# lowc1012/tensorflow-distributed-example

Measured on AMD Instinct MI355X. Metric: images/sec (whole node) MNIST CNN at 1/2/4/8 MI355X; step time ms, higher is better.
Workload: dtype fp32; 1 GPU; model=mnist_cnn, global_batch=64, per_gpu_batch=64, parallelism=dp1, replicas=1, replicas_per_process=1, distinct_devices=1, graphs_per_execution=1, steps_per_execution=3, warmup_steps_run=6360, optimizer=SGD(lr=0.001), plan=fused_convnet, allreduce=none, hipgraph=True, grad_buckets=1, optimizer_placement=in_step_kernels

## Files before the change

### csrc/include/tde_convnet.h

```cpp
#pragma once
#include "tde_optim.h"
#include "tde_xgmi.h"

namespace tde {
namespace cnet {

constexpr int CC = 32;
constexpr int HD = 64;
constexpr int NW = 16;

struct FwdArgs {
  const float* x; const float* wc; const float* bc;
  const void* W1; int ldw1;
  float* hpre;
  void* Pt; int ldPt;
  uint64_t* amax; int lda;
  int B, H, W;
  long long* stamps;
  int w1_rows;
  const int* pend;
  const float *gwc, *gbc, *mwc, *mbc, *vwc, *vbc;
  const long long* iterations;
  OptHyper h;
  unsigned long long* inc_iter;
  int hrep; long long hrep_stride;
  int grep; long long grep_stride;
  unsigned long long* fly_count;
  const float *hsrc_w2, *hsrc_b2, *hsrc_b1;
  float* hsnap;
  int hC;
};

__device__ __forceinline__ void fwd_snap_head(const FwdArgs& a, int nthreads) {
  if (!a.hsnap || blockIdx.x != 0 || blockIdx.y != 0) return;
  const int C = a.hC, n = HD + HD * C + C;
  for (int i = threadIdx.x; i < n; i += nthreads) {
    float v;
    if (i < HD) v = a.hsrc_b1 ? a.hsrc_b1[i] : 0.f;
    else if (i < HD + HD * C) v = a.hsrc_w2[i - HD];
    else v = a.hsrc_b2[i - HD - HD * C];
    a.hsnap[i] = v;
  }
}

constexpr int XR = 6, XW = 32;
__host__ __device__ constexpr int fwd_istride(int W) { return XR * W + ((2 - (XR * W) % 64) + 64) % 64; }
constexpr int kConvW = CC * 10;
constexpr int kXrBytes = 64 * (XR * XW + 64) * 4;

__device__ __forceinline__ void fwd_stage_x(const FwdArgs& a, float* xr, int b0, int py0, int nrows, int nthreads) {
  const int W = a.W, H = a.H;
  const int istride = fwd_istride(W);
  const int n4 = nrows * W / 4;
  constexpr int kU = 8;
  for (int i0 = threadIdx.x; i0 < 64 * n4; i0 += kU * nthreads) {
    float4 v[kU];
#pragma unroll
    for (int u = 0; u < kU; ++u) {
      const int i = i0 + u * nthreads, bl = i / n4, q = i - bl * n4;
      v[u] = float4{0.f, 0.f, 0.f, 0.f};
      if (i < 64 * n4 && b0 + bl < a.B)
        v[u] = *reinterpret_cast<const float4*>(a.x + (size_t)(b0 + bl) * H * W + (size_t)(2 * py0) * W + q * 4);
    }
#pragma unroll
    for (int u = 0; u < kU; ++u) {
      const int i = i0 + u * nthreads, bl = i / n4, q = i - bl * n4;
      if (i < 64 * n4) {
        float2* d2 = reinterpret_cast<float2*>(xr + bl * istride + q * 4);
        d2[0] = float2{v[u].x, v[u].y};
        d2[1] = float2{v[u].z, v[u].w};
      }
    }
  }
}

__device__ __forceinline__ void fwd_stage_conv(const FwdArgs& a, float* wcs, int nthreads) {
  for (int i = threadIdx.x; i < kConvW; i += nthreads) {
    const bool isb = i >= 9 * CC;
    const int j = isb ? i - 9 * CC : i;
    float w = isb ? a.bc[j] : a.wc[j];
    if (a.pend) {
      const float* gp = isb ? a.gbc + j : a.gwc + j;
      float gv[kMaxGrep];
#pragma unroll
      for (int r = 0; r < kMaxGrep; ++r) gv[r] = (r == 0 || r < a.grep) ? gp[r * a.grep_stride] : 0.f;
      float g = gv[0];
#pragma unroll
      for (int r = 1; r < kMaxGrep; ++r) g += gv[r];
      float m = 0.f, v = 0.f;
      if (a.h.kind != kOptSGD) m = isb ? a.mbc[j] : a.mwc[j];
      if (a.h.kind == kOptAdam) v = isb ? a.vbc[j] : a.vwc[j];
      const long long t = a.h.kind == kOptAdam ? *a.iterations : 0;
      if (*a.pend) w = opt_step(a.h, opt_lr_t(a.h, t), w, g, m, v);
    }
    wcs[i] = w;
  }
}

struct ConvW8 {
  float4 wlo[9], whi[9], blo, bhi;
  __device__ __forceinline__ void load(const float* wcs, int c0) {
#pragma unroll
    for (int t = 0; t < 9; ++t) {
      wlo[t] = *reinterpret_cast<const float4*>(wcs + t * CC + c0);
      whi[t] = *reinterpret_cast<const float4*>(wcs + t * CC + c0 + 4);
    }
    blo = *reinterpret_cast<const float4*>(wcs + 9 * CC + c0);
    bhi = *reinterpret_cast<const float4*>(wcs + 9 * CC + c0 + 4);
  }
};

__device__ __forceinline__ float f4get(float4 q, int k) { return k == 0 ? q.x : (k == 1 ? q.y : (k == 2 ? q.z : q.w)); }

__device__ __forceinline__ void conv_pool8(const float* xb, int W, const ConvW8& cw, float out[8], uint64_t& packed) {
  float patch[16];
#pragma unroll
  for (int r = 0; r < 4; ++r) {
    const float2 u = *reinterpret_cast<const float2*>(xb + r * W);
    const float2 v = *reinterpret_cast<const float2*>(xb + r * W + 2);
    patch[r * 4 + 0] = u.x; patch[r * 4 + 1] = u.y; patch[r * 4 + 2] = v.x; patch[r * 4 + 3] = v.y;
  }
  packed = 0;
#pragma unroll
  for (int cc = 0; cc < 8; ++cc) {
    float wt[9];
#pragma unroll
    for (int t = 0; t < 9; ++t) wt[t] = f4get(cc < 4 ? cw.wlo[t] : cw.whi[t], cc & 3);
    const float bcv = f4get(cc < 4 ? cw.blo : cw.bhi, cc & 3);
    float best = -3.0e38f;
    int bi = 0;
#pragma unroll
    for (int q = 0; q < 4; ++q) {
      const int dy = q >> 1, dx = q & 1;
      float z = bcv;
#pragma unroll
      for (int ky = 0; ky < 3; ++ky)
#pragma unroll
        for (int kx = 0; kx < 3; ++kx) z = fmaf(patch[(dy + ky) * 4 + dx + kx], wt[ky * 3 + kx], z);
      if (z > best) { best = z; bi = q; }
    }
    out[cc] = fmaxf(best, 0.f);
    packed |= (uint64_t)(best > 0.f ? (unsigned)bi : 0xFFu) << (8 * cc);
  }
}

struct BwdArgs {
  const float* x; const uint64_t* amax; int lda;
  const float* hpre;
  float* hzero;
  int hrep; long long hrep_stride;
  float* cpart;
  const float* b1; const float* W2; const float* b2; int C; int pre_relu;
  const int* labels;
  float scale;
  float* metrics;
// ... 17 lines not shown
  int* pend_set;
  XgPush push;
};

template <int NPER>
struct FlatPrefetch {
  int e[NPER];
  float w[NPER], g[NPER], m[NPER], v[NPER];
  __device__ __forceinline__ void load(const FlatApply& f, int tid, int nt) {
#pragma unroll
    for (int k = 0; k < NPER; ++k) {
      int idx = tid + k * nt;
      e[k] = -1;
      for (int r = 0; r < f.nr; ++r) {
        if (idx < f.n[r]) {
          e[k] = f.lo[r] + idx;
          break;
        }
        idx -= f.n[r];
      }
      w[k] = g[k] = m[k] = v[k] = 0.f;
      if (e[k] >= 0) {
        w[k] = f.w[e[k]];
        g[k] = flat_grad(f, e[k]);
        if (f.h.kind != kOptSGD) m[k] = f.m[e[k]];
        if (f.h.kind == kOptAdam) v[k] = f.v[e[k]];
      }
    }
  }
  __device__ __forceinline__ void apply(const FlatApply& f, long long t) {
    const float lr_t = opt_lr_t(f.h, t);
#pragma unroll
    for (int k = 0; k < NPER; ++k) {
      if (e[k] < 0) continue;
      f.w[e[k]] = opt_step(f.h, lr_t, w[k], g[k], m[k], v[k]);
      flat_grad_zero(f, e[k]);
      if (f.h.kind != kOptSGD) f.m[e[k]] = m[k];
      if (f.h.kind == kOptAdam) f.v[e[k]] = v[k];
    }
  }
};

__device__ __forceinline__ f32x4 mfma_f32x4(float a, float b, f32x4 c) {
  return __builtin_amdgcn_mfma_f32_16x16x4f32(a, b, c, 0, 0, 0);
}

constexpr int HS = HD + 4;
constexpr int DLS = 17, W2S = 17;
constexpr int kHeadScratch = 64 * HS * 4 + 12 * 64 * 4 * 4 + 64 * DLS * 4;
struct HeadLds {
  float* hs;
  float* part;
  float* dls;
  float* w2s;
  float* b2s;
  int* labs;
  __device__ __forceinline__ static HeadLds carve(unsigned char* scratch, unsigned char* w2, unsigned char* b2,
                                                  unsigned char* lab) {
    HeadLds l;
    l.hs = reinterpret_cast<float*>(scratch);
    l.part = reinterpret_cast<float*>(scratch + 64 * HS * 4);
    l.dls = reinterpret_cast<float*>(scratch + 64 * HS * 4 + 12 * 64 * 4 * 4);
    l.w2s = reinterpret_cast<float*>(w2);
    l.b2s = reinterpret_cast<float*>(b2);
    l.labs = reinterpret_cast<int*>(lab);
    return l;
  }
};
constexpr int kW2Bytes = HD * W2S * 4, kB2Bytes = 16 * 4, kLabBytes = 64 * 4;

__device__ __forceinline__ void head_load_w2(const BwdArgs& a, const HeadLds& l, int tid) {
  const int u = tid >> 4, c = tid & 15;
  l.w2s[u * W2S + c] = c < a.C ? a.W2[u * a.C + c] : 0.f;
  if (tid < 16) l.b2s[tid] = tid < a.C ? a.b2[tid] : 0.f;
}

__device__ __forceinline__ void zero_other_parity(const BwdArgs& a, int tid) {
  const int n4 = (int)(((a.hrep - 1) * a.hrep_stride + (long long)a.B * HD) / 4);
  const int per = (n4 + gridDim.x - 1) / gridDim.x, beg = blockIdx.x * per;
  const int end = min(n4, beg + per);
  for (int i = beg + tid; i < end; i += 1024) reinterpret_cast<float4*>(a.hzero)[i] = float4{0.f, 0.f, 0.f, 0.f};
}

__device__ __forceinline__ float4 load_hpre(const BwdArgs& a, int row, int c4) {
  constexpr int kMaxRep = 8;
  if (a.hrep > kMaxRep) {
    float4 s = {0.f, 0.f, 0.f, 0.f};
    for (int r = 0; r < a.hrep; ++r) {
      const float4 v = *reinterpret_cast<const float4*>(a.hpre + (size_t)r * a.hrep_stride + (size_t)row * HD + c4);
      s.x += v.x; s.y += v.y; s.z += v.z; s.w += v.w;
    }
    return s;
  }
  float4 v[kMaxRep];
#pragma unroll
  for (int r = 0; r < kMaxRep; ++r)
    v[r] = r < a.hrep ? *reinterpret_cast<const float4*>(a.hpre + (size_t)r * a.hrep_stride + (size_t)row * HD + c4)
                      : float4{0.f, 0.f, 0.f, 0.f};
  float4 s = v[0];
#pragma unroll
  for (int r = 1; r < kMaxRep; ++r) {
    s.x += v[r].x; s.y += v[r].y; s.z += v[r].z; s.w += v[r].w;
  }
  return s;
}

__device__ __forceinline__ void head_stage(const BwdArgs& a, float4 hv, float4 b1v, int hr, int hc4, int nb,
                                           float* hs) {
  float4 h = float4{hv.x + b1v.x, hv.y + b1v.y, hv.z + b1v.z, hv.w + b1v.w};
  if (a.pre_relu) h = float4{fmaxf(h.x, 0.f), fmaxf(h.y, 0.f), fmaxf(h.z, 0.f), fmaxf(h.w, 0.f)};
  if (hr >= nb) h = float4{0.f, 0.f, 0.f, 0.f};
  *reinterpret_cast<float4*>(hs + hr * HS + hc4) = h;
}

__device__ __forceinline__ void head_logits_ce(const BwdArgs& a, int nb, const HeadLds& l, int lane, int wave,
                                               float& la, float& ca, float& na) {
  const int fr = lane & 15, fq = lane >> 4, C = a.C;
  f32x4 lg = {0.f, 0.f, 0.f, 0.f};
  {
    const int rt = wave & 3, kq = wave >> 2;
#pragma unroll
    for (int k = kq * 16; k < kq * 16 + 16; k += 4)
      lg = mfma_f32x4(l.hs[(rt * 16 + fr) * HS + k + fq], l.w2s[(k + fq) * W2S + fr], lg);
    if (kq > 0) *reinterpret_cast<f32x4*>(l.part + (((kq - 1) * 4 + rt) * 64 + lane) * 4) = lg;
  }
  lds_barrier();
  if (wave < 4) {
    const int rt = wave;
#pragma unroll
    for (int q = 0; q < 3; ++q) {
      const f32x4 pv = *reinterpret_cast<const f32x4*>(l.part + ((q * 4 + rt) * 64 + lane) * 4);
      lg[0] += pv[0]; lg[1] += pv[1]; lg[2] += pv[2]; lg[3] += pv[3];
    }
#pragma unroll
    for (int i = 0; i < 4; ++i) {
      const int r = rt * 16 + fq * 4 + i;
      const bool valid = r < nb;
      const bool cv = fr < C;
      const float z = cv ? lg[i] + l.b2s[fr] : -3.0e38f;
      const float m = row16_max(z);
      const float e = cv ? __expf(z - m) : 0.f;
      const float s = row16_sum(e);
      const float pr = e / s;
      const int label = l.labs[r];
      const int amx = row16_min(cv && z == m ? fr : 64);
      const float zl = __shfl(z, (lane & ~15) | (label & 15), 64);
      if (valid && fr == 0) {
        la += __logf(s) + m - zl;
        ca += (amx == label) ? 1.f : 0.f;
        na += 1.f;
      }
      l.dls[r * DLS + fr] = (valid && cv) ? (pr - (fr == label ? 1.f : 0.f)) * a.scale : 0.f;
    }
  }
  lds_barrier();
}

__device__ __forceinline__ f32x4 head_dh(const BwdArgs& a, int nb, const HeadLds& l, int lane, int wave) {
  const int fr = lane & 15, fq = lane >> 4, rt = wave >> 2, ut = wave & 3;
  f32x4 gh = {0.f, 0.f, 0.f, 0.f};
#pragma unroll
  for (int k = 0; k < 16; k += 4)
    gh = mfma_f32x4(l.dls[(rt * 16 + fr) * DLS + k + fq], l.w2s[(ut * 16 + fr) * W2S + k + fq], gh);
  const int j = ut * 16 + fr;
#pragma unroll
  for (int i = 0; i < 4; ++i) {
    const int r = rt * 16 + fq * 4 + i;
    if ((a.pre_relu && !(l.hs[r * HS + j] > 0.f)) || r >= nb) gh[i] = 0.f;
  }
  return gh;
}

template <int MODE>
__device__ __forceinline__ void head_workgroup(const BwdArgs& a, const HeadLds& l, float* db1p) {
  const int lane = threadIdx.x & 63, wave = threadIdx.x >> 6, tid = threadIdx.x;
  const int fr = lane & 15, fq = lane >> 4, C = a.C;
  const int hr = tid >> 4, hc4 = (tid & 15) * 4;
  const float4 b1v = a.b1 ? *reinterpret_cast<const float4*>(a.b1 + hc4) : float4{0.f, 0.f, 0.f, 0.f};

  long long e[4] = {-1, -1, -1, -1};
  if (wave < 4 && fr < C) {
#pragma unroll
    for (int i = 0; i < 4; ++i) e[i] = a.off_w2 + (long long)(wave * 16 + fq * 4 + i) * C + fr;
  } else if (wave == 4 && fq == 0 && fr < C) {
    e[0] = a.off_b2 + fr;
  } else if (wave == 5 && a.off_b1 >= 0) {
    e[0] = a.off_b1 + lane;
  }
  float hwv[4] = {0.f, 0.f, 0.f, 0.f}, hmv[4] = {0.f, 0.f, 0.f, 0.f}, hvv[4] = {0.f, 0.f, 0.f, 0.f};
  long long t_it = 0;
  FlatPrefetch<1> cp;
  int cpend = 0;
  if (MODE != 0) {
    t_it = *a.iterations;
#pragma unroll
    for (int i = 0; i < 4; ++i) {
      if (e[i] < 0) continue;
      hwv[i] = a.hw[e[i]];
      if (MODE == 2 && a.h.kind != kOptSGD) hmv[i] = a.hm[e[i]];
      if (MODE == 2 && a.h.kind == kOptAdam) hvv[i] = a.hv[e[i]];
    }
    if (a.commit.nr > 0) {
      cpend = *a.commit.pend;
      cp.load(a.commit, tid, 1024);
    }
  }

  f32x4 gw = {0.f, 0.f, 0.f, 0.f};
  float db1acc = 0.f, db2acc = 0.f, la = 0.f, ca = 0.f, na = 0.f;
  for (int b0 = 0; b0 < a.B; b0 += 64) {
    const int nb = min(64, a.B - b0);
    float4 hv = {0.f, 0.f, 0.f, 0.f};
    if (hr < nb) hv = load_hpre(a, b0 + hr, hc4);
    const int lab = (tid < nb) ? a.labels[b0 + tid] : 0;
    head_stage(a, hv, b1v, hr, hc4, nb, l.hs);
    if (tid < 64) l.labs[tid] = lab;
    lds_barrier();
    head_logits_ce(a, nb, l, lane, wave, la, ca, na);
    const f32x4 gh = head_dh(a, nb, l, lane, wave);
    db1acc += (gh[0] + gh[1]) + (gh[2] + gh[3]);
    if (wave < 4) {
#pragma unroll
      for (int k = 0; k < 64; k += 4) gw = mfma_f32x4(l.hs[(k + fq) * HS + wave * 16 + fr], l.dls[(k + fq) * DLS + fr], gw);
    } else if (wave == 4) {
#pragma unroll 4
      for (int r = fq * 16; r < fq * 16 + 16; ++r) db2acc += l.dls[r * DLS + fr];
    }
    lds_barrier();
  }
  db1acc += __shfl_xor(db1acc, 16, 64);
  db1acc += __shfl_xor(db1acc, 32, 64);
  if (fq == 0) db1p[(wave >> 2) * 64 + (wave & 3) * 16 + fr] = db1acc;
  db2acc += __shfl_xor(db2acc, 16, 64);
  db2acc += __shfl_xor(db2acc, 32, 64);
  if (wave < 4) {
    la = rows4_sum(la);
    ca = rows4_sum(ca);
    na = rows4_sum(na);
    if (a.metrics && lane == 0 && na > 0.f) {
      atomicAdd(a.metrics + 0, la);
      atomicAdd(a.metrics + 1, ca);
      atomicAdd(a.metrics + 2, na);
    }
  }
  lds_barrier();
  float gv[4] = {0.f, 0.f, 0.f, 0.f};
  float* gdst[4] = {nullptr, nullptr, nullptr, nullptr};
  if (wave < 4 && fr < C) {
#pragma unroll
    for (int i = 0; i < 4; ++i) {
      gv[i] = gw[i];
      gdst[i] = a.dW2 ? a.dW2 + (size_t)(wave * 16 + fq * 4 + i) * C + fr : nullptr;
    }
  } else if (wave == 4 && fq == 0 && fr < C) {
    gv[0] = db2acc;
    gdst[0] = a.db2 ? a.db2 + fr : nullptr;
  } else if (wave == 5 && a.b1) {
    gv[0] = (db1p[lane] + db1p[64 + lane]) + (db1p[128 + lane] + db1p[192 + lane]);
    gdst[0] = a.db1 ? a.db1 + lane : nullptr;
  }
  if (MODE == 0) {
#pragma unroll
    for (int i = 0; i < 4; ++i)
      if (gdst[i]) *gdst[i] += gv[i];
    stamp(a.stamps, 7);
    return;
  }
  const float lr_t = opt_lr_t(a.h, t_it);
#pragma unroll
  for (int i = 0; i < 4; ++i) {
    if (e[i] < 0) continue;
    float m = hmv[i], v = hvv[i];
    a.hw[e[i]] = opt_step(a.h, lr_t, hwv[i], gv[i], m, v);
    if (MODE == 2 && a.h.kind != kOptSGD) a.hm[e[i]] = m;
    if (MODE == 2 && a.h.kind == kOptAdam) a.hv[e[i]] = v;
  }
  if (cpend) cp.apply(a.commit, t_it - 1);
  if (tid == 0) {
    if (cpend) *a.commit.pend = 0;
    if (cpend && a.commit.count) atomicAdd(a.commit.count, 1ull);
    if (a.pend_set) *a.pend_set = 1;
    if (a.iter_prev) *a.iter_prev = t_it;
  }
  stamp(a.stamps, 7);
}

__device__ __forceinline__ void conv_grad_reduce(const BwdArgs& a, const f32x4 accr[2], float* red, int lane, int wave) {
  const int fr = lane & 15, fq = lane >> 4, tid = threadIdx.x;
#pragma unroll
  for (int ct = 0; ct < 2; ++ct)
#pragma unroll
    for (int r = 0; r < 4; ++r) red[((size_t)wave * 16 + fq * 4 + r) * CC + ct * 16 + fr] = accr[ct][r];
  lds_barrier();
  if (tid < 10 * CC) {
    const int tap = tid / CC, c = tid - tap * CC;
    float s = 0.f;
#pragma unroll
    for (int w = 0; w < NW; ++w) s += red[((size_t)w * 16 + tap) * CC + c];
    if (a.cpart) a.cpart[(size_t)blockIdx.x * 10 * CC + tid] = s;
    else {
      const long long ro = a.crep > 1 ? (long long)(blockIdx.x % a.crep) * a.crep_stride : 0;
      if (tap < 9) {
        if (a.dwc) atomicAdd(a.dwc + ro + tap * CC + c, s);
      } else if (a.dbc) {
        atomicAdd(a.dbc + ro + c, s);
      }
    }
  }
}

}
}


struct TdeStepOpt {
  int kind;
  float lr, mom, b1, b2, eps;
  float *w, *g, *m, *v;
  const long long* iterations;
  int* pend;
  int grep; long long grep_stride;
  unsigned long long* fly_count;
  const float *hsrc_w2, *hsrc_b2, *hsrc_b1;
  float* hsnap;
  int hC;
};

struct TdeBwdOpt {
  int kind;
  float lr, mom, b1, b2, eps;
  float *w, *m, *v;
  long long off_w1, off_w2, off_b2, off_b1;
  void* W1c; int ldw1c;
  const long long* iterations;
  long long* iter_prev;
  tde::FlatApply commit;
  int* pend_set;
  int crep; long long crep_stride;
};

namespace tde {
namespace cnet {

inline OptHyper hyper_of(const TdeStepOpt* o) { return OptHyper{o->kind, o->lr, o->mom, o->b1, o->b2, o->eps}; }
inline bool opt_ok(const TdeStepOpt* o) {
  return o->w && o->g && o->iterations && (o->kind == kOptSGD || o->m) && (o->kind != kOptAdam || o->v) &&
         (!o->hsnap || (o->hsrc_w2 && o->hsrc_b2 && o->hC >= 1 && o->hC <= 16 && !((uintptr_t)o->hsnap & 15)));
}

inline void fill_fwd_opt(FwdArgs& a, const TdeStepOpt* opt, long long off_wc, long long off_bc, long long* inc_iter,
                         int hrep, long long hrep_stride) {
  a.inc_iter = (unsigned long long*)inc_iter;
  a.hrep = hrep > 0 ? hrep : 1;
  a.hrep_stride = hrep_stride;
  if (opt) {
    a.pend = opt->pend;
    a.gwc = opt->g + off_wc;
    a.gbc = opt->g + off_bc;
// ... 95 lines not shown
```

### csrc/kernels/convnet_f32.hip

```cpp
#include "tde_convnet.h"

namespace tde {
using namespace cnet;

constexpr int FG = 4;
constexpr int FB = 16;
constexpr int AS32 = 168;
constexpr int GS32 = 72;
constexpr int DPS32 = 40;
static_assert(FG == 4 && FB == 16, "the forward's lane maps are written for 4 positions x 16 images");

__host__ __device__ constexpr int fwd32_istride(int W) { return XR * W + ((4 - (XR * W) % 64) + 64) % 64; }
constexpr int kXr32Bytes = FB * (XR * XW + 64) * 4;
constexpr int kFwd32Lds = FB * AS32 * 4 + kXr32Bytes + kConvW * 4;

__device__ __forceinline__ int k8_col(int fq, int i) { return fq * 8 + 4 * ((i + fq) & 1); }
__device__ __forceinline__ int k16_col(int fq, int i) { return fq * 16 + 4 * ((i + fq) & 3); }

__device__ __forceinline__ void fwd32_stage_x(const FwdArgs& a, float* xr, int b0, int py0, int nrows) {
  const int W = a.W, H = a.H;
  const int istride = fwd32_istride(W);
  const int n4 = nrows * W / 4;
  constexpr int kU = 3;
  for (int i0 = threadIdx.x; i0 < FB * n4; i0 += kU * 256) {
    float4 v[kU];
#pragma unroll
    for (int u = 0; u < kU; ++u) {
      const int i = i0 + u * 256, bl = i / n4, q = i - bl * n4;
      v[u] = float4{0.f, 0.f, 0.f, 0.f};
      if (i < FB * n4 && b0 + bl < a.B)
        v[u] = *reinterpret_cast<const float4*>(a.x + (size_t)(b0 + bl) * H * W + (size_t)(2 * py0) * W + q * 4);
    }
#pragma unroll
    for (int u = 0; u < kU; ++u) {
      const int i = i0 + u * 256, bl = i / n4, q = i - bl * n4;
      if (i < FB * n4) *reinterpret_cast<float4*>(xr + bl * istride + q * 4) = v[u];
    }
  }
}

__global__ __launch_bounds__(256) void convnet32_fwd_kernel(FwdArgs a) {
  constexpr int NT = 256;
  extern __shared__ __attribute__((aligned(16))) unsigned char fsm[];
  float* As = reinterpret_cast<float*>(fsm);
  float* xr = reinterpret_cast<float*>(fsm + FB * AS32 * 4);
  float* wcs = reinterpret_cast<float*>(fsm + FB * AS32 * 4 + kXr32Bytes);
  stamp(a.stamps, 0);
  if (a.inc_iter && blockIdx.x == 0 && blockIdx.y == 0 && threadIdx.x == 0) atomicAdd(a.inc_iter, 1ull);
  if (a.fly_count && a.pend && blockIdx.x == 0 && blockIdx.y == 0 && threadIdx.x == 0 && *a.pend)
    atomicAdd(a.fly_count, 1ull);
  fwd_snap_head(a, NT);
  const int lane = threadIdx.x & 63, wave = __builtin_amdgcn_readfirstlane(threadIdx.x >> 6);
  const int fr = lane & 15, fq = lane >> 4;
  const int W = a.W, H = a.H;
  const int Wp = (W - 2) / 2, Hp = (H - 2) / 2, P = Hp * Wp;
  const int p0 = blockIdx.x * FG;
  const int b0 = blockIdx.y * FB;
  const int py0 = p0 / Wp;
  const int nrows = min(XR, H - 2 * py0);
  const float* W1 = reinterpret_cast<const float*>(a.W1);
  float* Pt = reinterpret_cast<float*>(a.Pt);

  const int nt = wave;
  float wfr[FG][8];
#pragma unroll
  for (int ks = 0; ks < FG; ++ks) {
    const int kp = p0 + ks;
#pragma unroll
    for (int i = 0; i < 2; ++i)
#pragma unroll
      for (int j = 0; j < 4; ++j)
        wfr[ks][4 * i + j] = kp < P ? W1[(size_t)(kp * CC + k8_col(fq, i) + j) * a.ldw1 + nt * 16 + fr] : 0.f;
  }
  fwd32_stage_x(a, xr, b0, py0, nrows);
  fwd_stage_conv(a, wcs, NT);
  stamp(a.stamps, 1);
  lds_barrier();

  const int cg = wave, c0 = cg * 8;
  ConvW8 cw;
  cw.load(wcs, c0);
  const int p = p0 + fq, b = b0 + fr;
  const bool pok = p < P, bok = b < a.B;
  float out[8];
  if (bok && pok) {
    const int py = p / Wp, px = p - py * Wp;
    uint64_t packed;
    conv_pool8(xr + fr * fwd32_istride(W) + (2 * (py - py0)) * W + 2 * px, W, cw, out, packed);
    if (a.amax) a.amax[((size_t)p * (CC / 8) + cg) * a.lda + b] = packed;
  } else {
#pragma unroll
    for (int cc = 0; cc < 8; ++cc) out[cc] = 0.f;
  }
  if (pok && Pt && (bok || b < a.ldPt)) {
#pragma unroll
    for (int cc = 0; cc < 8; ++cc) Pt[(size_t)(p * CC + c0 + cc) * a.ldPt + b] = out[cc];
  }
  {
    float* dst = As + fr * AS32 + fq * CC + c0;
    *reinterpret_cast<float4*>(dst) = float4{out[0], out[1], out[2], out[3]};
    *reinterpret_cast<float4*>(dst + 4) = float4{out[4], out[5], out[6], out[7]};
  }
  stamp(a.stamps, 2);
  lds_barrier();
  stamp(a.stamps, 3);

  float* const hrow = a.hpre + (size_t)(blockIdx.x % a.hrep) * a.hrep_stride;
  f32x4 acc[FG];
#pragma unroll
  for (int ks = 0; ks < FG; ++ks) acc[ks] = f32x4{0.f, 0.f, 0.f, 0.f};
#pragma unroll
  for (int i = 0; i < 2; ++i) {
    float4 av[FG];
#pragma unroll
    for (int ks = 0; ks < FG; ++ks)
      av[ks] = *reinterpret_cast<const float4*>(As + fr * AS32 + ks * CC + k8_col(fq, i));
#pragma unroll
    for (int e = 0; e < 4; ++e)
#pragma unroll
      for (int ks = 0; ks < FG; ++ks) acc[ks] = mfma_f32x4(f4get(av[ks], e), wfr[ks][4 * i + e], acc[ks]);
  }
#pragma unroll
  for (int r = 0; r < 4; ++r) {
    const int row = b0 + fq * 4 + r;
    const float s = ((acc[0][r] + acc[1][r]) + acc[2][r]) + acc[3][r];
    if (row < a.B) atomicAdd(hrow + (size_t)row * HD + nt * 16 + fr, s);
  }
  stamp(a.stamps, 4);
}

constexpr int kG32 = 0;
constexpr int kGt32 = kG32 + 64 * GS32 * 4;
constexpr int kW1s32 = kGt32 + 64 * GS32 * 4;
constexpr int kPts32 = kW1s32 + 32 * GS32 * 4;
constexpr int kXs32 = kPts32 + 32 * GS32 * 4;
constexpr int kAm32 = kXs32 + 64 * 16 * 4;
constexpr int kR32 = kAm32 + 64 * CC;
constexpr int kRBytes = kHeadScratch > NW * 16 * CC * 4 ? kHeadScratch : NW * 16 * CC * 4;
static_assert(64 * DPS32 * 4 <= kRBytes, "dP exceeds the shared scratch");
constexpr int kW2s32 = kR32 + kRBytes;
constexpr int kB2s32 = kW2s32 + kW2Bytes;
constexpr int kLab32 = kB2s32 + kB2Bytes;
constexpr int kBwd32Lds = kLab32 + kLabBytes;
static_assert(kBwd32Lds <= 160 * 1024, "backward LDS exceeds a CU");

template <int MODE>
__global__ __launch_bounds__(1024) void convnet32_bwd_kernel(BwdArgs a) {
  extern __shared__ __attribute__((aligned(16))) unsigned char smem[];
  float* Gs = reinterpret_cast<float*>(smem + kG32);
  float* Gts = reinterpret_cast<float*>(smem + kGt32);
  float* W1s = reinterpret_cast<float*>(smem + kW1s32);
  float* Pts = reinterpret_cast<float*>(smem + kPts32);
  float* xs = reinterpret_cast<float*>(smem + kXs32);
  uint8_t* am = smem + kAm32;
  float* dps = reinterpret_cast<float*>(smem + kR32);
  const HeadLds hl = HeadLds::carve(smem + kR32, smem + kW2s32, smem + kB2s32, smem + kLab32);
  stamp(a.stamps, 0);
  const int W = a.W, H = a.H;
  const int lane = threadIdx.x & 63, wave = threadIdx.x >> 6, tid = threadIdx.x;
  const int fr = lane & 15, fq = lane >> 4;
  const float* W1 = reinterpret_cast<const float*>(a.W1);
  const float* Pt = reinterpret_cast<const float*>(a.Pt);

  const int u2 = tid >> 4, c2 = tid & 15;
  const float w2v = c2 < a.C ? a.W2[u2 * a.C + c2] : 0.f;
  const float b2v = (tid < 16 && tid < a.C) ? a.b2[tid] : 0.f;
  zero_other_parity(a, tid);
  if (blockIdx.x == gridDim.x - 1) {
    hl.w2s[u2 * W2S + c2] = w2v;
    if (tid < 16) hl.b2s[tid] = b2v;
    head_workgroup<MODE>(a, hl, Gs);
    return;
  }

  const int Wp = (W - 2) / 2;
  const int p = blockIdx.x;
  const int py = p / Wp, px = p - py * Wp;
  const int hr = tid >> 4, hc4 = (tid & 15) * 4;
  const float4 b1v = a.b1 ? *reinterpret_cast<const float4*>(a.b1 + hc4) : float4{0.f, 0.f, 0.f, 0.f};
  const bool dw_wave = wave >= 8;
  const int v8 = wave & 7;

  f32x4 accw = {0.f, 0.f, 0.f, 0.f};
  f32x4 accr[2] = {{0.f, 0.f, 0.f, 0.f}, {0.f, 0.f, 0.f, 0.f}};

  f32x4 mp = {0.f, 0.f, 0.f, 0.f}, vp = {0.f, 0.f, 0.f, 0.f};
  long long t_it = 0;
  if (MODE != 0) {
    t_it = *a.iterations;
    if (MODE == 2 && dw_wave) {
      const int rt = v8 >> 2, nt = v8 & 3;
#pragma unroll
      for (int r = 0; r < 4; ++r) {
        const size_t e = (size_t)(p * CC + rt * 16 + fq * 4 + r) * HD + nt * 16 + fr;
        if (a.h.kind != kOptSGD) mp[r] = a.m1[e];
        if (a.h.kind == kOptAdam) vp[r] = a.v1[e];
      }
    }
  }

  const float2 w1v = *reinterpret_cast<const float2*>(W1 + (size_t)(p * CC + (tid >> 5)) * a.ldw1 + (tid & 31) * 2);

  for (int b0 = 0; b0 < a.B; b0 += 64) {
    const int nb = min(64, a.B - b0);
    float4 hv = {0.f, 0.f, 0.f, 0.f};
    if (hr < nb) hv = load_hpre(a, b0 + hr, hc4);
    const int lab = (tid < nb) ? a.labels[b0 + tid] : 0;
    float2 ptv;
    {
      const int r = tid >> 5, c = (tid & 31) * 2;
      const float* src = Pt + (size_t)(p * CC + r) * a.ldPt + b0 + c;
      ptv.x = c < nb ? src[0] : 0.f;
      ptv.y = c + 1 < nb ? src[1] : 0.f;
    }
    float4 xv = {0.f, 0.f, 0.f, 0.f};
    uint64_t amv = ~0ull;
    if (tid < 256) {
      const int bl = tid >> 2, r = tid & 3;
      if (bl < nb) {
        const float2* row = reinterpret_cast<const float2*>(a.x + (size_t)(b0 + bl) * H * W + (2 * py + r) * W + 2 * px);
        const float2 u = row[0], t = row[1];
        xv = float4{u.x, u.y, t.x, t.y};
      }
      const int cg = tid >> 6, bb = tid & 63;
      if (bb < nb) amv = a.amax[((size_t)p * (CC / 8) + cg) * a.lda + b0 + bb];
    }
    stamp(a.stamps, 1);
    if (b0 == 0) {
      hl.w2s[u2 * W2S + c2] = w2v;
      if (tid < 16) hl.b2s[tid] = b2v;
      *reinterpret_cast<float2*>(W1s + (tid >> 5) * GS32 + (tid & 31) * 2) = w1v;
    }
    head_stage(a, hv, b1v, hr, hc4, nb, hl.hs);
    if (tid < 64) hl.labs[tid] = lab;
    {
      const int r = tid >> 5, c = (tid & 31) * 2;
      *reinterpret_cast<float2*>(Pts + r * GS32 + c) = ptv;
    }
    if (tid < 256) {
      const int bl = tid >> 2, r = tid & 3;
      *reinterpret_cast<float4*>(xs + bl * 16 + r * 4) = xv;
      const int cg = tid >> 6, bb = tid & 63;
      *reinterpret_cast<uint64_t*>(am + bb * CC + cg * 8) = amv;
    }
    lds_barrier();
    {
      float la = 0.f, ca = 0.f, na = 0.f;
      head_logits_ce(a, nb, hl, lane, wave, la, ca, na);
      const f32x4 gh = head_dh(a, nb, hl, lane, wave);
      const int rt = wave >> 2, j = (wave & 3) * 16 + fr;
#pragma unroll
      for (int i = 0; i < 4; ++i) Gs[(rt * 16 + fq * 4 + i) * GS32 + j] = gh[i];
      *reinterpret_cast<float4*>(Gts + j * GS32 + rt * 16 + fq * 4) = float4{gh[0], gh[1], gh[2], gh[3]};
    }
    lds_barrier();
    stamp(a.stamps, 2);

    {
      const float* Ab = dw_wave ? Pts + ((v8 >> 2) * 16 + fr) * GS32 : Gs + ((v8 >> 1) * 16 + fr) * GS32;
      const float* Bb = dw_wave ? Gts + ((v8 & 3) * 16 + fr) * GS32 : W1s + ((v8 & 1) * 16 + fr) * GS32;
      f32x4 acc = dw_wave ? accw : f32x4{0.f, 0.f, 0.f, 0.f};
#pragma unroll
      for (int i = 0; i < 4; ++i) {
        const float4 av = *reinterpret_cast<const float4*>(Ab + k16_col(fq, i));
        const float4 bv = *reinterpret_cast<const float4*>(Bb + k16_col(fq, i));
        acc = mfma_f32x4(av.x, bv.x, acc);
        acc = mfma_f32x4(av.y, bv.y, acc);
        acc = mfma_f32x4(av.z, bv.z, acc);
        acc = mfma_f32x4(av.w, bv.w, acc);
      }
      if (dw_wave) {
        accw = acc;
      } else {
        const int mt = v8 >> 1, ct = v8 & 1;
#pragma unroll
        for (int r = 0; r < 4; ++r) dps[(mt * 16 + fq * 4 + r) * DPS32 + ct * 16 + fr] = acc[r];
      }
    }
    lds_barrier();
    stamp(a.stamps, 3);

    {
      const int tap = fr, ky = tap / 3, kx = tap - ky * 3, qy = fq >> 1, qx = fq & 1;
#pragma unroll
      for (int s = 0; s < 4; ++s) {
        const int bl = wave * 4 + s;
        const float xa = tap < 9 ? xs[bl * 16 + (qy + ky) * 4 + qx + kx] : (tap == 9 ? 1.f : 0.f);
#pragma unroll
        for (int ct = 0; ct < 2; ++ct) {
          const int c = ct * 16 + fr;
          const float d = am[bl * CC + c] == (unsigned)fq ? dps[bl * DPS32 + c] : 0.f;
          accr[ct] = mfma_f32x4(xa, d, accr[ct]);
        }
      }
    }
    lds_barrier();
  }
  stamp(a.stamps, 4);

  if (dw_wave) {
    const int rt = v8 >> 2, nt = v8 & 3;
    const int col = nt * 16 + fr;
    if (MODE != 0) {
      const float lr_t = opt_lr_t(a.h, t_it);
#pragma unroll
      for (int r = 0; r < 4; ++r) {
        const int row = rt * 16 + fq * 4 + r;
        const size_t e = (size_t)(p * CC + row) * HD + col;
        float m = mp[r], v = vp[r];
        a.w1[e] = opt_step(a.h, lr_t, W1s[row * GS32 + col], accw[r], m, v);
        if (MODE == 2 && a.h.kind != kOptSGD) a.m1[e] = m;
        if (MODE == 2 && a.h.kind == kOptAdam) a.v1[e] = v;
      }
    } else if (a.push.nranks > 0) {
#pragma unroll
      for (int r = 0; r < 4; ++r) W1s[(rt * 16 + fq * 4 + r) * GS32 + col] = accw[r];
    } else {
#pragma unroll
      for (int r = 0; r < 4; ++r) a.dW1[(size_t)(p * CC + rt * 16 + fq * 4 + r) * HD + col] = accw[r];
    }
  }
  conv_grad_reduce(a, accr, dps, lane, wave);
  if (MODE == 0 && a.push.nranks > 0 && tid < CC * HD / 4) {
    const int parity = (int)((*a.push.epoch + 1u) & 1u);
    const int row = tid >> 4, c4 = (tid & 15) * 4;
    xg_push_store4(a.push, parity, a.push.off + (long long)(p * CC + row) * HD + c4,
                   *reinterpret_cast<const float4*>(W1s + row * GS32 + c4));
    xg_push_drain();
  }
  stamp(a.stamps, 5);
}

}

using namespace tde;
using namespace tde::cnet;

TDE_API int tde_convnet_fwd_f32(const float* x, const float* wc, const float* bc, const float* W1, int ldw1,
                                float* hpre, float* Pt, int ldPt, void* amax, int lda, int B, int H, int W,
                                long long* stamps, const TdeStepOpt* opt, long long off_wc, long long off_bc,
                                long long* inc_iter, int hrep, long long hrep_stride, hipStream_t stream) {
  if ((W & 3) || W > XW || ((W - 2) / 2) < 4 || ldw1 != HD || (Pt && (ldPt & 7)) || (amax && lda < B)) return -1;
  if (((uintptr_t)wc | (uintptr_t)bc | (uintptr_t)W1) & 15) return -2;
  if (opt && (!opt_ok(opt) || !opt->pend)) return -4;
  const int P = ((H - 2) / 2) * ((W - 2) / 2);
  const int by = ((Pt && ldPt > B ? ldPt : B) + FB - 1) / FB;
  FwdArgs a{x, wc, bc, W1, ldw1, hpre, Pt, ldPt, (uint64_t*)amax, lda, B, H, W, stamps};
  fill_fwd_opt(a, opt, off_wc, off_bc, inc_iter, hrep, hrep_stride);
  const dim3 grid((P + FG - 1) / FG, by);
  convnet32_fwd_kernel<<<grid, 256, kFwd32Lds, stream>>>(a);
  TDE_LAUNCH_CHECK();
  return 0;
}

TDE_API int tde_convnet_bwd_f32(const float* x, const void* amax, int lda, const float* hpre, float* hzero,
                                int hrep, long long hrep_stride, const float* b1, const float* W2, const float* b2,
                                int C, int pre_relu, const int* labels, float scale, float* metrics, const float* W1,
                                int ldw1, const float* Pt, int ldPt, float* dW1, float* dwc, float* dbc, float* dW2,
                                float* db2, float* db1, int B, int H, int W, long long* stamps, const TdeBwdOpt* opt,
                                float* cpart, const XgPush* push, int crep, long long crep_stride,
                                hipStream_t stream) {
  if (ldw1 != HD || ((uintptr_t)W1 & 15) || ((uintptr_t)Pt & 7)) return -1;
  if (push && push->nranks > 0 &&
      (opt || push->nranks > kXgMaxRanks || push->L <= 0 || (push->L & 3) || (push->off & 3) || !push->epoch))
    return -7;
  if (opt && opt->w + opt->off_w1 != W1) return -3;
  BwdArgs a;
  const int rc = fill_bwd(a, x, amax, lda, hpre, hzero, hrep, hrep_stride, b1, W2, b2, C, pre_relu, labels, scale,
                          metrics, W1, ldw1, Pt, ldPt, dW1, dwc, dbc, dW2, db2, db1, B, H, W, stamps, opt);
  if (rc) return rc;
  a.cpart = cpart;
  a.w1r_out = nullptr;
  a.w1c_out = nullptr;
  if (push) a.push = *push;
  if (!opt && crep > 1) {
    a.crep = crep;
    a.crep_stride = crep_stride;
  }
  const int P = ((H - 2) / 2) * ((W - 2) / 2);
  static bool attr_set = false;
  if (!attr_set) {
    (void)hipFuncSetAttribute((const void*)convnet32_bwd_kernel<0>, hipFuncAttributeMaxDynamicSharedMemorySize, kBwd32Lds);
// ... 19 lines not shown
```

Measured before the change: 2.619 million images/sec.

## Hoist and batch global loads ahead of use in fused convnet fwd/bwd kernels

Restructures the forward and backward fp32 convnet kernels so that global loads are issued early and unconditionally, with clamped indices, into register structs. These cover input rows, conv weights and optimizer state, the head snapshot, hpre replicas, labels, Pt, x and amax. Masking is applied after the loads arrive, and an opaque thread-id trick keeps the compiler from rematerialising addresses. hpre replicas are summed through a switch over the replica count into templated, fully unrolled loads. The goal is to overlap memory latency in this latency-bound small-batch step, at the cost of more registers and some redundant loads.

```diff
diff --git a/csrc/include/tde_convnet.h b/csrc/include/tde_convnet.h
--- a/csrc/include/tde_convnet.h
+++ b/csrc/include/tde_convnet.h
@@ -43,6 +43,31 @@
   }
 }
 
+template <int NT>
+struct SnapHead {
+  static constexpr int N = (HD + HD * 16 + 16 + NT - 1) / NT;
+  float v[N];
+  __device__ __forceinline__ static bool mine(const FwdArgs& a) { return a.hsnap && blockIdx.x == 0 && blockIdx.y == 0; }
+  __device__ __forceinline__ void issue(const FwdArgs& a) {
+    const int C = a.hC, n = HD + HD * C + C;
+#pragma unroll
+    for (int k = 0; k < N; ++k) {
+      const int i = min((int)threadIdx.x + k * NT, n - 1);
+      const float* src = i < HD ? (a.hsrc_b1 ? a.hsrc_b1 + i : a.hsrc_w2 + i)
+                                : (i < HD + HD * C ? a.hsrc_w2 + (i - HD) : a.hsrc_b2 + (i - HD - HD * C));
+      v[k] = *src;
+    }
+  }
+  __device__ __forceinline__ void store(const FwdArgs& a) const {
+    const int C = a.hC, n = HD + HD * C + C;
+#pragma unroll
+    for (int k = 0; k < N; ++k) {
+      const int i = (int)threadIdx.x + k * NT;
+      if (i < n) a.hsnap[i] = (i < HD && !a.hsrc_b1) ? 0.f : v[k];
+    }
+  }
+};
+
 constexpr int XR = 6, XW = 32;
 __host__ __device__ constexpr int fwd_istride(int W) { return XR * W + ((2 - (XR * W) % 64) + 64) % 64; }
 constexpr int kConvW = CC * 10;
@@ -71,6 +96,40 @@
         d2[1] = float2{v[u].z, v[u].w};
       }
     }
+  }
+}
+
+struct ConvOperand {
+  float w, g[kMaxGrep], m, v;
+  __device__ __forceinline__ void issue(const FwdArgs& a, int i) {
+    const bool isb = i >= 9 * CC;
+    const int j = isb ? i - 9 * CC : i;
+    const float* wp = isb ? a.bc + j : a.wc + j;
+    w = *wp;
+    if (a.pend) {
+      const float* gp = isb ? a.gbc + j : a.gwc + j;
+#pragma unroll
+      for (int r = 0; r < kMaxGrep; ++r) g[r] = gp[min(r, a.grep - 1) * a.grep_stride];
+      m = *(a.h.kind != kOptSGD ? (isb ? a.mbc + j : a.mwc + j) : wp);
+      v = *(a.h.kind == kOptAdam ? (isb ? a.vbc + j : a.vwc + j) : wp);
+    }
+  }
+  __device__ __forceinline__ float finish(const FwdArgs& a, int pend, long long iterations) {
+    if (!a.pend) return w;
+    float gs = g[0];
+#pragma unroll
+    for (int r = 1; r < kMaxGrep; ++r) gs += r < a.grep ? g[r] : 0.f;
+    const long long t = a.h.kind == kOptAdam ? iterations : 0;
+    float ms = a.h.kind != kOptSGD ? m : 0.f, vs = a.h.kind == kOptAdam ? v : 0.f;
+    return pend ? opt_step(a.h, opt_lr_t(a.h, t), w, gs, ms, vs) : w;
+  }
+};
+__device__ __forceinline__ void conv_flags_issue(const FwdArgs& a, int& pend, long long& iterations) {
+  pend = 0;
+  iterations = 0;
+  if (a.pend) {
+    pend = *a.pend;
+    iterations = *a.iterations;
   }
 }
 
@@ -254,16 +313,56 @@
   for (int i = beg + tid; i < end; i += 1024) reinterpret_cast<float4*>(a.hzero)[i] = float4{0.f, 0.f, 0.f, 0.f};
 }
 
+__device__ __forceinline__ int opaque_tid() {
+  int t = threadIdx.x;
+  asm volatile("" : "+v"(t));
+  return t;
+}
+
+constexpr int kMaxRep = 8;
+template <int N>
+struct HpreRep {
+  float4 v[N];
+  __device__ __forceinline__ void issue(const BwdArgs& a, int row, int c4) {
+#pragma unroll
+    for (int r = 0; r < N; ++r)
+      v[r] = *reinterpret_cast<const float4*>(a.hpre + (size_t)min(r, a.hrep - 1) * a.hrep_stride + (size_t)row * HD + c4);
+  }
+  __device__ __forceinline__ float4 sum(const BwdArgs& a) const {
+    float4 s = v[0];
+#pragma unroll
+    for (int r = 1; r < N; ++r) {
+      const bool on = r < a.hrep;
+      s.x += on ? v[r].x : 0.f; s.y += on ? v[r].y : 0.f; s.z += on ? v[r].z : 0.f; s.w += on ? v[r].w : 0.f;
+    }
+    return s;
+  }
+};
+__device__ __forceinline__ float4 load_hpre_loop(const BwdArgs& a, int row, int c4) {
+  float4 s = {0.f, 0.f, 0.f, 0.f};
+  for (int r = 0; r < a.hrep; ++r) {
+    const float4 v = *reinterpret_cast<const float4*>(a.hpre + (size_t)r * a.hrep_stride + (size_t)row * HD + c4);
+    s.x += v.x; s.y += v.y; s.z += v.z; s.w += v.w;
+  }
+  return s;
+}
+template <int N>
+__device__ __forceinline__ float4 load_hpre_n(const BwdArgs& a, int row, int c4) {
+  HpreRep<N> h;
+  h.issue(a, row, c4);
+  return h.sum(a);
+}
+__device__ __forceinline__ float4 load_hpre_sw(const BwdArgs& a, int row, int c4) {
+  if (a.hrep > kMaxRep) return load_hpre_loop(a, row, c4);
+  switch (a.hrep) {
+    case 1: return load_hpre_n<1>(a, row, c4);
+    case 2: return load_hpre_n<2>(a, row, c4);
+    case 3: case 4: return load_hpre_n<4>(a, row, c4);
+    default: return load_hpre_n<8>(a, row, c4);
+  }
+}
 __device__ __forceinline__ float4 load_hpre(const BwdArgs& a, int row, int c4) {
-  constexpr int kMaxRep = 8;
-  if (a.hrep > kMaxRep) {
-    float4 s = {0.f, 0.f, 0.f, 0.f};
-    for (int r = 0; r < a.hrep; ++r) {
-      const float4 v = *reinterpret_cast<const float4*>(a.hpre + (size_t)r * a.hrep_stride + (size_t)row * HD + c4);
-      s.x += v.x; s.y += v.y; s.z += v.z; s.w += v.w;
-    }
-    return s;
-  }
+  if (a.hrep > kMaxRep) return load_hpre_loop(a, row, c4);
   float4 v[kMaxRep];
 #pragma unroll
   for (int r = 0; r < kMaxRep; ++r)
@@ -343,34 +442,34 @@
   return gh;
 }
 
-template <int MODE>
+__device__ __forceinline__ long long head_var(const BwdArgs& a, int tid, int i) {
+  const int lane = tid & 63, wave = tid >> 6, fr = lane & 15, fq = lane >> 4, C = a.C;
+  if (wave < 4 && fr < C) return a.off_w2 + (long long)(wave * 16 + fq * 4 + i) * C + fr;
+  if (i == 0 && wave == 4 && fq == 0 && fr < C) return a.off_b2 + fr;
+  if (i == 0 && wave == 5 && a.off_b1 >= 0) return a.off_b1 + lane;
+  return -1;
+}
+
+template <int MODE, bool LEAN = false>
 __device__ __forceinline__ void head_workgroup(const BwdArgs& a, const HeadLds& l, float* db1p) {
   const int lane = threadIdx.x & 63, wave = threadIdx.x >> 6, tid = threadIdx.x;
   const int fr = lane & 15, fq = lane >> 4, C = a.C;
-  const int hr = tid >> 4, hc4 = (tid & 15) * 4;
-  const float4 b1v = a.b1 ? *reinterpret_cast<const float4*>(a.b1 + hc4) : float4{0.f, 0.f, 0.f, 0.f};
-
-  long long e[4] = {-1, -1, -1, -1};
-  if (wave < 4 && fr < C) {
-#pragma unroll
-    for (int i = 0; i < 4; ++i) e[i] = a.off_w2 + (long long)(wave * 16 + fq * 4 + i) * C + fr;
-  } else if (wave == 4 && fq == 0 && fr < C) {
-    e[0] = a.off_b2 + fr;
-  } else if (wave == 5 && a.off_b1 >= 0) {
-    e[0] = a.off_b1 + lane;
-  }
+  const float4 b1v = a.b1 ? *reinterpret_cast<const float4*>(a.b1 + (tid & 15) * 4) : float4{0.f, 0.f, 0.f, 0.f};
+
   float hwv[4] = {0.f, 0.f, 0.f, 0.f}, hmv[4] = {0.f, 0.f, 0.f, 0.f}, hvv[4] = {0.f, 0.f, 0.f, 0.f};
   long long t_it = 0;
   FlatPrefetch<1> cp;
   int cpend = 0;
   if (MODE != 0) {
     t_it = *a.iterations;
+    const int tl = LEAN ? opaque_tid() : (int)threadIdx.x;
 #pragma unroll
     for (int i = 0; i < 4; ++i) {
-      if (e[i] < 0) continue;
-      hwv[i] = a.hw[e[i]];
-      if (MODE == 2 && a.h.kind != kOptSGD) hmv[i] = a.hm[e[i]];
-      if (MODE == 2 && a.h.kind == kOptAdam) hvv[i] = a.hv[e[i]];
+      const long long e = head_var(a, tl, i);
+      if (e < 0) continue;
+      hwv[i] = a.hw[e];
+      if (MODE == 2 && a.h.kind != kOptSGD) hmv[i] = a.hm[e];
+      if (MODE == 2 && a.h.kind == kOptAdam) hvv[i] = a.hv[e];
     }
     if (a.commit.nr > 0) {
       cpend = *a.commit.pend;
@@ -382,8 +481,11 @@
   float db1acc = 0.f, db2acc = 0.f, la = 0.f, ca = 0.f, na = 0.f;
   for (int b0 = 0; b0 < a.B; b0 += 64) {
     const int nb = min(64, a.B - b0);
+    const int tid = LEAN ? opaque_tid() : (int)threadIdx.x;
+    const int lane = tid & 63, wave = tid >> 6, fr = lane & 15, fq = lane >> 4;
+    const int hr = tid >> 4, hc4 = (tid & 15) * 4;
     float4 hv = {0.f, 0.f, 0.f, 0.f};
-    if (hr < nb) hv = load_hpre(a, b0 + hr, hc4);
+    if (hr < nb) hv = LEAN ? load_hpre_sw(a, b0 + hr, hc4) : load_hpre(a, b0 + hr, hc4);
     const int lab = (tid < nb) ? a.labels[b0 + tid] : 0;
     head_stage(a, hv, b1v, hr, hc4, nb, l.hs);
     if (tid < 64) l.labs[tid] = lab;
@@ -439,13 +541,15 @@
     return;
   }
   const float lr_t = opt_lr_t(a.h, t_it);
+  const int tl = LEAN ? opaque_tid() : (int)threadIdx.x;
 #pragma unroll
   for (int i = 0; i < 4; ++i) {
-    if (e[i] < 0) continue;
+    const long long e = head_var(a, tl, i);
+    if (e < 0) continue;
     float m = hmv[i], v = hvv[i];
-    a.hw[e[i]] = opt_step(a.h, lr_t, hwv[i], gv[i], m, v);
-    if (MODE == 2 && a.h.kind != kOptSGD) a.hm[e[i]] = m;
-    if (MODE == 2 && a.h.kind == kOptAdam) a.hv[e[i]] = v;
+    a.hw[e] = opt_step(a.h, lr_t, hwv[i], gv[i], m, v);
+    if (MODE == 2 && a.h.kind != kOptSGD) a.hm[e] = m;
+    if (MODE == 2 && a.h.kind == kOptAdam) a.hv[e] = v;
   }
   if (cpend) cp.apply(a.commit, t_it - 1);
   if (tid == 0) {
diff --git a/csrc/kernels/convnet_f32.hip b/csrc/kernels/convnet_f32.hip
--- a/csrc/kernels/convnet_f32.hip
+++ b/csrc/kernels/convnet_f32.hip
@@ -17,27 +17,32 @@
 __device__ __forceinline__ int k8_col(int fq, int i) { return fq * 8 + 4 * ((i + fq) & 1); }
 __device__ __forceinline__ int k16_col(int fq, int i) { return fq * 16 + 4 * ((i + fq) & 3); }
 
-__device__ __forceinline__ void fwd32_stage_x(const FwdArgs& a, float* xr, int b0, int py0, int nrows) {
-  const int W = a.W, H = a.H;
-  const int istride = fwd32_istride(W);
-  const int n4 = nrows * W / 4;
-  constexpr int kU = 3;
-  for (int i0 = threadIdx.x; i0 < FB * n4; i0 += kU * 256) {
-    float4 v[kU];
+struct Fwd32X {
+  static constexpr int kU = 3;
+  static_assert(FB * XR * XW / 4 <= kU * 256, "one pass of the workgroup stages the rows");
+  float4 v[kU];
+  __device__ __forceinline__ void issue(const FwdArgs& a, int b0, int py0, int nrows) {
+    const int W = a.W, H = a.H;
+    const int n4 = nrows * W / 4;
 #pragma unroll
     for (int u = 0; u < kU; ++u) {
-      const int i = i0 + u * 256, bl = i / n4, q = i - bl * n4;
+      const int i = threadIdx.x + u * 256, bl = i / n4, q = i - bl * n4;
       v[u] = float4{0.f, 0.f, 0.f, 0.f};
       if (i < FB * n4 && b0 + bl < a.B)
         v[u] = *reinterpret_cast<const float4*>(a.x + (size_t)(b0 + bl) * H * W + (size_t)(2 * py0) * W + q * 4);
     }
+  }
+  __device__ __forceinline__ void store(const FwdArgs& a, float* xr, int nrows) const {
+    const int W = a.W;
+    const int istride = fwd32_istride(W);
+    const int n4 = nrows * W / 4;
 #pragma unroll
     for (int u = 0; u < kU; ++u) {
-      const int i = i0 + u * 256, bl = i / n4, q = i - bl * n4;
+      const int i = threadIdx.x + u * 256, bl = i / n4, q = i - bl * n4;
       if (i < FB * n4) *reinterpret_cast<float4*>(xr + bl * istride + q * 4) = v[u];
     }
   }
-}
+};
 
 __global__ __launch_bounds__(256) void convnet32_fwd_kernel(FwdArgs a) {
   constexpr int NT = 256;
@@ -45,11 +50,11 @@
   float* As = reinterpret_cast<float*>(fsm);
   float* xr = reinterpret_cast<float*>(fsm + FB * AS32 * 4);
   float* wcs = reinterpret_cast<float*>(fsm + FB * AS32 * 4 + kXr32Bytes);
+  int pendv;
+  long long iterv;
+  conv_flags_issue(a, pendv, iterv);
   stamp(a.stamps, 0);
   if (a.inc_iter && blockIdx.x == 0 && blockIdx.y == 0 && threadIdx.x == 0) atomicAdd(a.inc_iter, 1ull);
-  if (a.fly_count && a.pend && blockIdx.x == 0 && blockIdx.y == 0 && threadIdx.x == 0 && *a.pend)
-    atomicAdd(a.fly_count, 1ull);
-  fwd_snap_head(a, NT);
   const int lane = threadIdx.x & 63, wave = __builtin_amdgcn_readfirstlane(threadIdx.x >> 6);
   const int fr = lane & 15, fq = lane >> 4;
   const int W = a.W, H = a.H;
@@ -61,19 +66,30 @@
   const float* W1 = reinterpret_cast<const float*>(a.W1);
   float* Pt = reinterpret_cast<float*>(a.Pt);
 
+  static_assert(kConvW > NT && kConvW <= NT + 64, "wave 0 holds the conv operands past the first NT");
+  Fwd32X xst;
+  xst.issue(a, b0, py0, nrows);
+  ConvOperand cv0, cv1;
+  cv0.issue(a, threadIdx.x);
+  if (wave == 0) cv1.issue(a, NT + min((int)threadIdx.x, kConvW - NT - 1));
+  SnapHead<NT> snap;
+  const bool snap_wg = SnapHead<NT>::mine(a);
+  if (snap_wg) snap.issue(a);
   const int nt = wave;
   float wfr[FG][8];
 #pragma unroll
   for (int ks = 0; ks < FG; ++ks) {
-    const int kp = p0 + ks;
+    const int kp = min(p0 + ks, P - 1);
 #pragma unroll
     for (int i = 0; i < 2; ++i)
 #pragma unroll
-      for (int j = 0; j < 4; ++j)
-        wfr[ks][4 * i + j] = kp < P ? W1[(size_t)(kp * CC + k8_col(fq, i) + j) * a.ldw1 + nt * 16 + fr] : 0.f;
-  }
-  fwd32_stage_x(a, xr, b0, py0, nrows);
-  fwd_stage_conv(a, wcs, NT);
+      for (int j = 0; j < 4; ++j) wfr[ks][4 * i + j] = W1[(size_t)(kp * CC + k8_col(fq, i) + j) * a.ldw1 + nt * 16 + fr];
+  }
+  xst.store(a, xr, nrows);
+  wcs[threadIdx.x] = cv0.finish(a, pendv, iterv);
+  if (wave == 0 && threadIdx.x < kConvW - NT) wcs[NT + threadIdx.x] = cv1.finish(a, pendv, iterv);
+  if (snap_wg) snap.store(a);
+  if (a.fly_count && pendv && blockIdx.x == 0 && blockIdx.y == 0 && threadIdx.x == 0) atomicAdd(a.fly_count, 1ull);
   stamp(a.stamps, 1);
   lds_barrier();
 
@@ -105,6 +121,10 @@
   lds_barrier();
   stamp(a.stamps, 3);
 
+#pragma unroll
+  for (int ks = 0; ks < FG; ++ks)
+#pragma unroll
+    for (int i = 0; i < 8; ++i) wfr[ks][i] = p0 + ks < P ? wfr[ks][i] : 0.f;
   float* const hrow = a.hpre + (size_t)(blockIdx.x % a.hrep) * a.hrep_stride;
   f32x4 acc[FG];
 #pragma unroll
@@ -144,6 +164,53 @@
 constexpr int kBwd32Lds = kLab32 + kLabBytes;
 static_assert(kBwd32Lds <= 160 * 1024, "backward LDS exceeds a CU");
 
+__device__ __forceinline__ void bwd32_ids(int& tid, int& lane, int& wave, int& fr, int& fq) {
+  const int t = opaque_tid();
+  tid = t;
+  lane = t & 63;
+  wave = t >> 6;
+  fr = lane & 15;
+  fq = lane >> 4;
+}
+
+struct Bwd32Chunk {
+  float4 hv;
+  int lab;
+  float2 ptv;
+  float4 xv;
+  uint64_t amv;
+};
+
+template <int NREP>
+__device__ __forceinline__ void bwd32_chunk_issue(const BwdArgs& a, int tid, int p, int py, int px, int b0, int nb,
+                                                  Bwd32Chunk& c) {
+  const int last = nb - 1;
+  const int hrow = b0 + min(tid >> 4, last), hc4 = (tid & 15) * 4;
+  HpreRep<(NREP > 0 ? NREP : 1)> h;
+  if (NREP > 0) h.issue(a, hrow, hc4);
+  c.lab = a.labels[b0 + min(tid, last)];
+  const int pc = (tid & 31) * 2;
+  c.ptv = *reinterpret_cast<const float2*>(reinterpret_cast<const float*>(a.Pt) + (size_t)(p * CC + (tid >> 5)) * a.ldPt +
+                                           b0 + min(pc, last & ~1));
+  c.xv = float4{0.f, 0.f, 0.f, 0.f};
+  c.amv = ~0ull;
+  if (tid < 256) {
+    const int bl = tid >> 2, r = tid & 3;
+    const float2* row = reinterpret_cast<const float2*>(a.x + (size_t)(b0 + min(bl, last)) * a.H * a.W +
+                                                        (2 * py + r) * a.W + 2 * px);
+    const float2 u = row[0], t = row[1];
+    c.xv = float4{u.x, u.y, t.x, t.y};
+    const int cg = tid >> 6, bb = tid & 63;
+    c.amv = a.amax[((size_t)p * (CC / 8) + cg) * a.lda + b0 + min(bb, last)];
+  }
+  c.hv = NREP > 0 ? h.sum(a) : load_hpre_loop(a, hrow, hc4);
+  if ((tid >> 2) >= nb) c.xv = float4{0.f, 0.f, 0.f, 0.f};
+  if ((tid & 63) >= nb) c.amv = ~0ull;
+  if (tid >= nb) c.lab = 0;
+  if (pc >= nb) c.ptv.x = 0.f;
+  if (pc + 1 >= nb) c.ptv.y = 0.f;
+}
+
 template <int MODE>
 __global__ __launch_bounds__(1024) void convnet32_bwd_kernel(BwdArgs a) {
   extern __shared__ __attribute__((aligned(16))) unsigned char smem[];
@@ -155,47 +222,44 @@
   uint8_t* am = smem + kAm32;
   float* dps = reinterpret_cast<float*>(smem + kR32);
   const HeadLds hl = HeadLds::carve(smem + kR32, smem + kW2s32, smem + kB2s32, smem + kLab32);
+  long long t_it = 0;
+  if (MODE == 2) t_it = *a.iterations;
+  const unsigned nwg = gridDim.x;
   stamp(a.stamps, 0);
-  const int W = a.W, H = a.H;
-  const int lane = threadIdx.x & 63, wave = threadIdx.x >> 6, tid = threadIdx.x;
-  const int fr = lane & 15, fq = lane >> 4;
+  const int W = a.W;
+  int tid, lane, wave, fr, fq;
+  bwd32_ids(tid, lane, wave, fr, fq);
   const float* W1 = reinterpret_cast<const float*>(a.W1);
-  const float* Pt = reinterpret_cast<const float*>(a.Pt);
-
-  const int u2 = tid >> 4, c2 = tid & 15;
-  const float w2v = c2 < a.C ? a.W2[u2 * a.C + c2] : 0.f;
-  const float b2v = (tid < 16 && tid < a.C) ? a.b2[tid] : 0.f;
+
+  float w2v, b2v;
+  {
+    const int u2 = tid >> 4, c2 = tid & 15;
+    w2v = a.W2[u2 * a.C + min(c2, a.C - 1)];
+    b2v = a.b2[min(c2, a.C - 1)];
+  }
   zero_other_parity(a, tid);
-  if (blockIdx.x == gridDim.x - 1) {
-    hl.w2s[u2 * W2S + c2] = w2v;
-    if (tid < 16) hl.b2s[tid] = b2v;
-    head_workgroup<MODE>(a, hl, Gs);
+  if (blockIdx.x == nwg - 1) {
+    hl.w2s[(tid >> 4) * W2S + (tid & 15)] = (tid & 15) < a.C ? w2v : 0.f;
+    if (tid < 16) hl.b2s[tid] = tid < a.C ? b2v : 0.f;
+    head_workgroup<MODE, true>(a, hl, Gs);
     return;
   }
 
   const int Wp = (W - 2) / 2;
   const int p = blockIdx.x;
   const int py = p / Wp, px = p - py * Wp;
-  const int hr = tid >> 4, hc4 = (tid & 15) * 4;
-  const float4 b1v = a.b1 ? *reinterpret_cast<const float4*>(a.b1 + hc4) : float4{0.f, 0.f, 0.f, 0.f};
-  const bool dw_wave = wave >= 8;
-  const int v8 = wave & 7;
-
+  const float4 b1v = *reinterpret_cast<const float4*>((a.b1 ? a.b1 : a.hpre) + (tid & 15) * 4);
   f32x4 accw = {0.f, 0.f, 0.f, 0.f};
   f32x4 accr[2] = {{0.f, 0.f, 0.f, 0.f}, {0.f, 0.f, 0.f, 0.f}};
 
   f32x4 mp = {0.f, 0.f, 0.f, 0.f}, vp = {0.f, 0.f, 0.f, 0.f};
-  long long t_it = 0;
-  if (MODE != 0) {
-    t_it = *a.iterations;
-    if (MODE == 2 && dw_wave) {
-      const int rt = v8 >> 2, nt = v8 & 3;
-#pragma unroll
-      for (int r = 0; r < 4; ++r) {
-        const size_t e = (size_t)(p * CC + rt * 16 + fq * 4 + r) * HD + nt * 16 + fr;
-        if (a.h.kind != kOptSGD) mp[r] = a.m1[e];
-        if (a.h.kind == kOptAdam) vp[r] = a.v1[e];
-      }
+  if (MODE == 2 && wave >= 8) {
+    const int rt = (wave & 7) >> 2, nt = wave & 3;
+#pragma unroll
+    for (int r = 0; r < 4; ++r) {
+      const size_t e = (size_t)(p * CC + rt * 16 + fq * 4 + r) * HD + nt * 16 + fr;
+      if (a.h.kind != kOptSGD) mp[r] = a.m1[e];
+      if (a.h.kind == kOptAdam) vp[r] = a.v1[e];
     }
   }
 
@@ -203,45 +267,33 @@
 
   for (int b0 = 0; b0 < a.B; b0 += 64) {
     const int nb = min(64, a.B - b0);
-    float4 hv = {0.f, 0.f, 0.f, 0.f};
-    if (hr < nb) hv = load_hpre(a, b0 + hr, hc4);
-    const int lab = (tid < nb) ? a.labels[b0 + tid] : 0;
-    float2 ptv;
-    {
-      const int r = tid >> 5, c = (tid & 31) * 2;
-      const float* src = Pt + (size_t)(p * CC + r) * a.ldPt + b0 + c;
-      ptv.x = c < nb ? src[0] : 0.f;
-      ptv.y = c + 1 < nb ? src[1] : 0.f;
-    }
-    float4 xv = {0.f, 0.f, 0.f, 0.f};
-    uint64_t amv = ~0ull;
+    bwd32_ids(tid, lane, wave, fr, fq);
+    const bool dw_wave = wave >= 8;
+    const int v8 = wave & 7;
+    Bwd32Chunk ck;
+    if (a.hrep > kMaxRep) bwd32_chunk_issue<0>(a, tid, p, py, px, b0, nb, ck);
+    else switch (a.hrep) {
+      case 1: bwd32_chunk_issue<1>(a, tid, p, py, px, b0, nb, ck); break;
+      case 2: bwd32_chunk_issue<2>(a, tid, p, py, px, b0, nb, ck); break;
+      case 3: case 4: bwd32_chunk_issue<4>(a, tid, p, py, px, b0, nb, ck); break;
+      default: bwd32_chunk_issue<8>(a, tid, p, py, px, b0, nb, ck); break;
+    }
+    stamp(a.stamps, 1);
+    const bool has_b1 = a.b1 && tid >= 0;
+    const float4 b1u = has_b1 ? b1v : float4{0.f, 0.f, 0.f, 0.f};
+    if (b0 == 0) {
+      hl.w2s[(tid >> 4) * W2S + (tid & 15)] = (tid & 15) < a.C ? w2v : 0.f;
+      if (tid < 16) hl.b2s[tid] = tid < a.C ? b2v : 0.f;
+      *reinterpret_cast<float2*>(W1s + (tid >> 5) * GS32 + (tid & 31) * 2) = w1v;
+    }
+    head_stage(a, ck.hv, b1u, tid >> 4, (tid & 15) * 4, nb, hl.hs);
+    if (tid < 64) hl.labs[tid] = ck.lab;
+    *reinterpret_cast<float2*>(Pts + (tid >> 5) * GS32 + (tid & 31) * 2) = ck.ptv;
     if (tid < 256) {
       const int bl = tid >> 2, r = tid & 3;
-      if (bl < nb) {
-        const float2* row = reinterpret_cast<const float2*>(a.x + (size_t)(b0 + bl) * H * W + (2 * py + r) * W + 2 * px);
-        const float2 u = row[0], t = row[1];
-        xv = float4{u.x, u.y, t.x, t.y};
-      }
+      *reinterpret_cast<float4*>(xs + bl * 16 + r * 4) = ck.xv;
       const int cg = tid >> 6, bb = tid & 63;
-      if (bb < nb) amv = a.amax[((size_t)p * (CC / 8) + cg) * a.lda + b0 + bb];
-    }
-    stamp(a.stamps, 1);
-    if (b0 == 0) {
-      hl.w2s[u2 * W2S + c2] = w2v;
-      if (tid < 16) hl.b2s[tid] = b2v;
-      *reinterpret_cast<float2*>(W1s + (tid >> 5) * GS32 + (tid & 31) * 2) = w1v;
-    }
-    head_stage(a, hv, b1v, hr, hc4, nb, hl.hs);
-    if (tid < 64) hl.labs[tid] = lab;
-    {
-      const int r = tid >> 5, c = (tid & 31) * 2;
-      *reinterpret_cast<float2*>(Pts + r * GS32 + c) = ptv;
-    }
-    if (tid < 256) {
-      const int bl = tid >> 2, r = tid & 3;
-      *reinterpret_cast<float4*>(xs + bl * 16 + r * 4) = xv;
-      const int cg = tid >> 6, bb = tid & 63;
-      *reinterpret_cast<uint64_t*>(am + bb * CC + cg * 8) = amv;
+      *reinterpret_cast<uint64_t*>(am + bb * CC + cg * 8) = ck.amv;
     }
     lds_barrier();
     {
@@ -298,6 +350,9 @@
   }
   stamp(a.stamps, 4);
 
+  bwd32_ids(tid, lane, wave, fr, fq);
+  const bool dw_wave = wave >= 8;
+  const int v8 = wave & 7;
   if (dw_wave) {
     const int rt = v8 >> 2, nt = v8 & 3;
     const int col = nt * 16 + fr;
```

Result: faster. 2.777 million images/sec (median of 6 runs) (+6.0%).
